# mkofinas/aether

Measured on AMD Instinct MI355X. Metric: edge-messages/sec (forward, electrostatic N=20 batch=128 per GPU), higher is better.
Workload: dtype f32; 1 GPU; electrostatic-2d-N20-B128; num_dims=2, nodes_per_graph=20, graphs_per_gpu=128, edges_per_gpu=48640, hidden=64, launch=hipgraph (10 steps per replay), parallelism=graphs sharded over 1 rank(s), no forward collective

## Files before the change

aether_amd/csrc/fused.h:

```cpp
#pragma once
#include "common.h"

#ifndef AETHER_SUMS_SELECT
#define AETHER_SUMS_SELECT 0
#endif
#ifndef AETHER_LATE_WAIT_FIRST
#define AETHER_LATE_WAIT_FIRST 0
#endif

namespace {

constexpr int FUSED_MAX_NODES = 32;
constexpr int FUSED_MAX_EDGES = 384;
constexpr int FUSED_MAX_TILES = FUSED_MAX_EDGES / 16;
constexpr int LDU = 2 * H + 8;

constexpr int FUSED_WIMG = SPLIT_WIMG;
constexpr int FUSED_CBLK = 768;
constexpr int CB_B1 = 0;
constexpr int CB_B2 = 64;
constexpr int CB_B3 = 128;
constexpr int CB_B4 = 256;
constexpr int CB_B1N = 320;
constexpr int CB_OB3 = 384;
constexpr int CB_OB6 = 448;
constexpr int CB_OW6 = 512;
template <int NW, int ROUNDS> struct FusedLds {
    static constexpr int WSZ = FUSED_WIMG;
    static constexpr int WA = 0;
    static constexpr int WB = WA + WSZ;
    static constexpr int CBLK = WB + WSZ;
    static constexpr int XBUF = CBLK + 2 * FUSED_CBLK;
    static constexpr int NBUF = XBUF + FUSED_MAX_NODES * LDW;
    static constexpr int PS = NBUF + FUSED_MAX_NODES * LDW;
    static constexpr int PR = PS + FUSED_MAX_NODES * LDW;
    static constexpr int NINFO = PR + FUSED_MAX_NODES * LDW;
    static constexpr int PART_ROWS = ROUNDS == 3 ? FUSED_MAX_NODES + FUSED_MAX_TILES : 2 * FUSED_MAX_NODES + 16;
    static constexpr int PART_SPARE = AETHER_SUMS_SELECT ? 1 : 0;
    static constexpr int PART = NINFO + FUSED_MAX_NODES * 24;
    static constexpr int ARRIVED = PART + (PART_ROWS + PART_SPARE) * LDW;
    static constexpr int SCRATCH = ARRIVED + 4;
    static constexpr int FEAT_ROWS = 16 * (ROUNDS < 2 ? ROUNDS : 2);
    static constexpr int SCRATCH_SIZE =
        NW * FEAT_ROWS * LDF > NW * 16 * LDST ? NW * FEAT_ROWS * LDF : NW * 16 * LDST;
    static constexpr int TOTAL = SCRATCH + SCRATCH_SIZE;
    static constexpr int FIELD_Z = SCRATCH;
    static constexpr int FIELD_H1 = FIELD_Z + FUSED_MAX_NODES * 24;
    static constexpr int FIELD_H2 = FIELD_H1 + FUSED_MAX_NODES * 32;
    static constexpr int FIELD_F = FIELD_H2 + FUSED_MAX_NODES * 32;
    static constexpr int FIELD_W = FIELD_F + FUSED_MAX_NODES * 4;
    static constexpr int FW0 = FIELD_W;
    static constexpr int FW2 = FW0 + 32 * 22;
    static constexpr int FW4 = FW2 + 32 * 32;
    static constexpr int FB = FW4 + 3 * 32;
    static constexpr int FEMB = FB + 68;
    static constexpr int FIELD_END = FEMB + 48;
    static constexpr int FEAT = SCRATCH;
    static constexpr int WSTAGE = SCRATCH;
    static constexpr int UBUF = SCRATCH;
    static constexpr int OBUF1 = SCRATCH;
    static constexpr int OBUF2 = SCRATCH + FUSED_MAX_NODES * LDW;
    static_assert(FIELD_END <= TOTAL, "field scratch");
    static_assert(UBUF + FUSED_MAX_NODES * LDU <= TOTAL, "ubuf");
    static_assert(OBUF2 + FUSED_MAX_NODES * LDW <= TOTAL, "obuf");
    static_assert(TOTAL * 4 <= 160 * 1024, "LDS budget");
};

constexpr int FUSED_NIMG_W3 = 2 * 8 * 2 * 64 * 4, FUSED_NIMG_W4 = 2 * 4 * 4 * 64 * 4, FUSED_NIMG_WS = 2 * 4 * 2 * 64 * 4;
constexpr int FUSED_NIMG_LAYER = FUSED_NIMG_W3 + FUSED_NIMG_W4 + 2 * FUSED_NIMG_WS;
constexpr int FUSED_WIMG_SET = 8 * FUSED_WIMG + 4 * FUSED_NIMG_LAYER + 4 * FUSED_CBLK;
constexpr int FUSED_SPLIT_BLOCKS = 8 + 4 * 6 + 1;
__device__ __host__ constexpr int fused_wimg_offset(int layer, int which) { return ((layer - 1) * 2 + which) * FUSED_WIMG; }
__device__ __host__ constexpr int fused_nimg_offset(int layer, int which) {
    return 8 * FUSED_WIMG + (layer - 1) * FUSED_NIMG_LAYER +
           (which == 0 ? 0 : which == 1 ? FUSED_NIMG_W3 : which == 2 ? FUSED_NIMG_W3 + FUSED_NIMG_W4 : FUSED_NIMG_W3 + FUSED_NIMG_W4 + FUSED_NIMG_WS);
}
__device__ __host__ constexpr int fused_cblk_offset(int layer) { return 8 * FUSED_WIMG + 4 * FUSED_NIMG_LAYER + (layer - 1) * FUSED_CBLK; }

__device__ __forceinline__ float fused_cblk_value(const AetherParams& P, int nd, int layer, int c) {
    if (c < CB_B2) return layer == 1 ? P.l1_msg_b0[c] : 0.0f;
    if (c < CB_B3) return (layer == 1 ? P.l1_msg_b2 : P.ln_msg_b2[layer - 2])[c - CB_B2];
    if (c < CB_B4) return (layer == 1 ? P.l1_upd_b0 : P.ln_upd_b0[layer - 2])[c - CB_B3];
    if (c < CB_B1N) return (layer == 1 ? P.l1_upd_b2 : P.ln_upd_b2[layer - 2])[c - CB_B4];
    if (c < CB_OB3) return (layer < 4 ? P.ln_msg_b0[layer - 1] : P.out_b0)[c - CB_B1N];
    if (layer < 4) return 0.0f;
    if (c < CB_OB6) return P.out_b3[c - CB_OB3];
    if (c < CB_OB6 + 4) return c - CB_OB6 < nd ? P.out_b6[c - CB_OB6] : 0.0f;
    if (c >= CB_OW6 && c < CB_OW6 + nd * H) return P.out_w6[c - CB_OW6];
    return 0.0f;
}

__device__ __forceinline__ void split_weights_block(const AetherParams& P, int f1, int nd, float* __restrict__ wimg, int block, int tid) {
    if (block == FUSED_SPLIT_BLOCKS - 1) {
        for (int idx = tid; idx < 4 * FUSED_CBLK; idx += 512)
            wimg[fused_cblk_offset(1) + idx] = fused_cblk_value(P, nd, idx / FUSED_CBLK + 1, idx % FUSED_CBLK);
        return;
    }
    if (block >= 8) {
        const int nbk = block - 8, layer = nbk / 6 + 1, part = nbk % 6;
        if (part < 2) {
            const float* w3 = layer == 1 ? P.l1_upd_w0 : P.ln_upd_w0[layer - 2];
            float* img = wimg + fused_nimg_offset(layer, 0);
#pragma unroll
            for (int j = 0; j < 2; ++j) {
                const int idx = tid + 512 * j, rr = 64 * part + (idx >> 4), cc = (idx & 15) * 4;
                stage_split4<8, 2>(img, rr, cc, ld4(w3 + (size_t)rr * H + cc));
            }
        } else if (part < 4) {
            const float* w4 = layer == 1 ? P.l1_upd_w2 : P.ln_upd_w2[layer - 2];
            float* img = wimg + fused_nimg_offset(layer, 1);
#pragma unroll
            for (int j = 0; j < 2; ++j) {
                const int idx = tid + 512 * j, rr = 32 * (part - 2) + (idx >> 5), cc = (idx & 31) * 4;
                stage_split4<4, 4>(img, rr, cc, ld4(w4 + (size_t)rr * (2 * H) + cc));
            }
        } else {
            const float* src = layer < 4 ? P.ln_msg_w0[layer - 1] + (part == 4 ? 0 : H) : (part == 4 ? P.out_w0 : P.out_w3);
            const int ld = layer < 4 ? 3 * H : H;
            float* img = wimg + fused_nimg_offset(layer, part - 2);
#pragma unroll
            for (int j = 0; j < 2; ++j) {
                const int idx = tid + 512 * j, rr = idx >> 4, cc = (idx & 15) * 4;
                stage_split4<4, 2>(img, rr, cc, ld4(src + (size_t)rr * ld + cc));
            }
        }
        return;
    }
    const int layer = block / 2 + 1, which = block & 1;
    float* img = wimg + fused_wimg_offset(layer, which);
    if (which == 0 && layer == 1) {
        const int r = tid >> 3, c0 = (tid & 7) * 4;
        f32x4 v;
#pragma unroll
        for (int b = 0; b < 4; ++b) v[b] = c0 + b < f1 ? P.l1_msg_w0[r * f1 + c0 + b] : 0.0f;
        stage_split4<4, 1>(img, r, c0, v);
        return;
    }
    const float* src;
    int ld;
    if (which == 0) { src = P.ln_msg_w0[layer - 2] + 2 * H; ld = 3 * H; }
    else { src = layer == 1 ? P.l1_msg_w2 : P.ln_msg_w2[layer - 2]; ld = H; }
#pragma unroll
    for (int j = 0; j < 2; ++j) {
        const int idx = tid + 512 * j, rr = idx >> 4, cc = (idx & 15) * 4;
        stage_split4<4, 2>(img, rr, cc, ld4(src + (size_t)rr * ld + cc));
    }
}

struct FusedDebug {
    float* nodeinfo; float* x[5]; float* e[4];
    float* n[4]; float* ps[3]; float* pr[3]; float* feat;
    int* flags;
    int* errword;
    const float* wimg;
    float* stamps;
    StepExtras step;
};
constexpr int FUSED_STAMPS = 512;

#ifdef AETHER_FUSED_STAMPS
// ... 84 lines not shown
    const int lane = threadIdx.x, i = lane & 15, q = lane >> 4;
    const int local = 16 * T.t + i;
    const bool valid = local < m;
    const int rcv = valid ? recv_s[eb + lorder[eb + local]] - wg.nb : -1;
    const int next = __shfl_down(rcv, 1, 16);
    const bool ends = valid && (i == 15 || next != rcv || local + 1 == na);
    const unsigned emask = (unsigned)__ballot(q == 0 && ends) & 0xFFFFu;
    const int second = (wg.partner >= 0 && local >= na) ? n : 0;
    const int myrow = rcv + T.t + second;
    const int j = lane & (FUSED_TREC - 1);
    unsigned w = 0;
#pragma unroll
    for (int b = 0; b < 4; ++b) {
        const int seg = 4 * (j - 2) + b;
        unsigned mm = emask;
        for (int t = 0; t < seg && mm != 0; ++t) mm &= mm - 1;
        const bool exists = seg >= 0 && seg < 16 && mm != 0;
        const int k = mm != 0 ? __ffs(mm) - 1 : 0;
        const int row = __shfl(myrow, k);
        w |= (exists ? (unsigned)row & 0xFFu : 0xFFu) << (8 * b);
    }
    if (j == 0) w = emask;
    if (j == 1) w = (unsigned)__popc(emask);
    if (j >= 6) w = 0;
    if (lane < FUSED_TREC) trec[(size_t)blockIdx.x * FUSED_TREC + lane] = w;
}

__device__ inline void graph_gtile(const int32_t* __restrict__ recv_s, int64_t n_edges, uint32_t* __restrict__ gsel,
                                   int64_t tile, int lane) {
    const int i = lane & 15, q = lane >> 4;
    const int64_t k = tile * 16 + i;
    const bool valid = k < n_edges;
    const int rcv = valid ? recv_s[k] : -1;
    const int prev = __shfl_up(rcv, 1, 16);
    const unsigned smask = (unsigned)__ballot(q == 0 && i > 0 && rcv != prev) & 0xFFFFu;
    const unsigned vmask = (unsigned)__ballot(q == 0 && valid) & 0xFFFFu;
    unsigned w = 0;
#pragma unroll
    for (int s4 = 0; s4 < 4; ++s4) {
        const int edge = 4 * s4 + q;
        const int seg_of_edge = __popc(smask & ((2u << edge) - 1u));
        if (((vmask >> edge) & 1u) && seg_of_edge == i) w |= 1u << s4;
    }
#pragma unroll
    for (int r4 = 0; r4 < 4; ++r4) {
        const int seg = 4 * q + r4;
        unsigned mm = smask;
        int s0 = 0;
        bool exists = true;
        for (int t = 0; t < seg; ++t) {
            if (mm == 0) { exists = false; break; }
            s0 = __ffs(mm) - 1;
            mm &= mm - 1;
        }
        const unsigned ok = (exists && ((vmask >> s0) & 1u)) ? 16u : 0u;
        w |= ((unsigned)s0 | ok) << (4 + 5 * r4);
    }
    gsel[(size_t)tile * 64 + lane] = w;
}

__global__ void __launch_bounds__(64)
k_graph_gtiles(const int32_t* __restrict__ recv_s, int64_t n_edges, uint32_t* __restrict__ gsel) {
    graph_gtile(recv_s, n_edges, gsel, (int64_t)blockIdx.x, threadIdx.x);
}

constexpr int GRAN_ROW = H * 8, GRAN_NODE = 3 * GRAN_ROW;
typedef unsigned int gran_u32x4 __attribute__((ext_vector_type(4)));

__device__ __forceinline__ auto gran_rsrc(int* flags, int goff, int vb, int nv) {
    return __builtin_amdgcn_make_buffer_rsrc(reinterpret_cast<char*>(flags) + goff + (int64_t)vb * GRAN_NODE, 0, nv * GRAN_NODE,
                                             0x00020000);
}

template <class Rsrc>
__device__ __forceinline__ void gran_publish(Rsrc rsrc, int row, int c0, int layer, f32x4 val) {
    const unsigned tag = (unsigned)layer;
    const gran_u32x4 g01 = {tag, __float_as_uint(val[0]), tag, __float_as_uint(val[1])};
    const gran_u32x4 g23 = {tag, __float_as_uint(val[2]), tag, __float_as_uint(val[3])};
    const int voff = row * GRAN_NODE + c0 * 8, soff = (layer - 1) * GRAN_ROW;
    __builtin_amdgcn_raw_buffer_store_b128(g01, rsrc, voff, soff, 16);
    __builtin_amdgcn_raw_buffer_store_b128(g23, rsrc, voff + 16, soff, 16);
}

template <class Rsrc, class LdsWord>
__device__ __forceinline__ void gran_receive(Rsrc rsrc, int layer, int nv, int n, int off, int lane, float* psb,
                                             LdsWord* arrived, int* errword) {
    constexpr int NL = 5;
    const int npieces = (nv - n) * (H / 2);
    const unsigned tag = (unsigned)(layer - 1);
    const int soff = (layer - 2) * GRAN_ROW;
    for (int base = 0; base < npieces; base += 64 * NL) {
        int src[NL];
#pragma unroll
        for (int j = 0; j < NL; ++j) {
            const int idx = base + 64 * j + lane, idc = idx < npieces ? idx : 0;
            int slot = idc >> 5;
            if (slot >= off) slot += n;
            src[j] = slot * GRAN_NODE + (idc & 31) * 16;
        }
        gran_u32x4 v[NL];
        unsigned spins = 0;
        unsigned long long t_first = 0;
        bool gave_up = false;
        for (;;) {
            asm volatile("" ::: "memory");
#pragma unroll
            for (int j = 0; j < NL; ++j) v[j] = __builtin_amdgcn_raw_buffer_load_b128(rsrc, src[j], soff, 16);
            __builtin_amdgcn_sched_barrier(0);
            __builtin_amdgcn_s_waitcnt(0x0F70);
            __builtin_amdgcn_sched_barrier(0);
            bool ok = true;
#pragma unroll
            for (int j = 0; j < NL; ++j) {
                asm volatile("" : "+v"(v[j]));
                ok = ok && v[j][0] == tag && v[j][2] == tag;
            }
            if (__all(ok)) break;
            __builtin_amdgcn_s_sleep(1);
            if ((++spins & 1023u) == 0) {
                const unsigned long long now = wall_clock64();
                if (t_first == 0) t_first = now;
                if (now - t_first <= 500000000ull) continue;
                if (lane == 0) {
                    if (errword) __hip_atomic_store(errword, 1, __ATOMIC_RELAXED, __HIP_MEMORY_SCOPE_SYSTEM);
                    arrived[1] = 1;
                }
                gave_up = true;
                break;
            }
        }
#pragma unroll
        for (int j = 0; j < NL; ++j) {
            if (base + 64 * j + lane < npieces) {
                const int row = src[j] / GRAN_NODE, c = ((src[j] % GRAN_NODE) >> 4) * 2;
                *reinterpret_cast<f32x2*>(psb + row * LDW + c) = f32x2{__uint_as_float(v[j][1]), __uint_as_float(v[j][3])};
            }
        }
        if (gave_up) break;
    }
}

template <class Rsrc>
__device__ __forceinline__ void gran_rearm(Rsrc rsrc, int nv, int n, int off, int t, int nthreads) {
    constexpr int PIECES = GRAN_NODE / 16;
    const gran_u32x4 zero = {0u, 0u, 0u, 0u};
    for (int idx = t; idx < (nv - n) * PIECES; idx += nthreads) {
        int slot = idx / PIECES;
        const int piece = idx - slot * PIECES;
        if (slot >= off) slot += n;
        __builtin_amdgcn_raw_buffer_store_b128(zero, rsrc, slot * GRAN_NODE + piece * 16, 0, 16);
    }
}

#ifndef AETHER_R3_DEFER
#define AETHER_R3_DEFER 0
#endif
template <int D, int NW, int ROUNDS, bool KEEP, bool GRAN = false>
__global__ void __launch_bounds__(NW * 64)
k_fused(AetherParams P, const float* __restrict__ x, const float* __restrict__ vel,
        const float* __restrict__ charges, const float* __restrict__ edge_attr_orig,
        const int32_t* __restrict__ perm, const int32_t* __restrict__ send_s,
        const int32_t* __restrict__ recv_s, const int32_t* __restrict__ rowptr,
        const FusedWG* __restrict__ wgdesc, const uint32_t* __restrict__ trec, const int4* __restrict__ ledge,
        const int32_t* __restrict__ nrange, FusedDebug dbg, float* __restrict__ out) {
    constexpr bool keep = KEEP;
    using NI = NodeInfo<D>;
    using L = FusedLds<NW, ROUNDS>;
    constexpr int THREADS = NW * 64;
    constexpr int FIN = 2 * D + 16;
    static_assert(NW == 8 || NW == 12, "waves 0-7 run the node phase; NW == 12 adds four waves that run step 3 (DESIGN.md 4.1)");
    static_assert(NW == 8 || (ROUNDS == 1 && !KEEP), "the 12-wave kernel owns one tile per wave and saves nothing for the backward");
    static_assert(!GRAN || NW == 12, "granules are the 12-wave kernel's hand-off");
    extern __shared__ __attribute__((aligned(16))) float smem[];
    float* wA = smem + L::WA;
    float* wB = smem + L::WB;
    const float* cblk = smem + L::CBLK;
    float* xbuf = smem + L::XBUF;
    float* nbuf = smem + L::NBUF;
    float* psb = smem + L::PS;
    float* prb = smem + L::PR;
    float* ninfo = smem + L::NINFO;
    float* part = smem + L::PART;

    const int tid = threadIdx.x, lane = tid & 63, wave = tid >> 6;
    const int i = lane & 15, q = lane >> 4;
    const FusedWG wg = wgdesc[blockIdx.x];
    const int vb = wg.vb, nv = wg.ve - wg.vb;
    const int nb = wg.nb, ne = wg.ne;
    const int n = ne - nb, off = nb - vb;
    const int eb = wg.eb, m = wg.m;
    const int n_tiles = (m + 15) >> 4;
    const int na = wg.na;
    typedef __attribute__((address_space(3))) volatile int lds_word;
    lds_word* arrived = (lds_word*)(smem + L::ARRIVED);
    if (tid == 0) { arrived[0] = 0; arrived[1] = 0; }
#ifdef AETHER_FUSED_STAMPS
    const unsigned long long t_entry = wall_clock64();
    const unsigned long long c_entry = __builtin_amdgcn_s_memtime();
#endif
    FUSED_STAMP(0);

    auto dma_images = [&](int layer_) {
        const int na_frag = layer_ == 1 ? 8 : 16, nw_frag = na_frag + 16;
        const int total = nw_frag + FUSED_CBLK / 256;
        const int wv = __builtin_amdgcn_readfirstlane(wave);
        __builtin_assume(wv >= 0 && wv < NW);
        const int g_img = fused_wimg_offset(layer_, 0), g_cb = fused_cblk_offset(layer_);
        const int l_cb = L::CBLK + (layer_ & 1) * FUSED_CBLK;
        constexpr int MAXF = (32 + FUSED_CBLK / 256 + NW - 1) / NW;
#pragma unroll
        for (int j = 0; j < MAXF; ++j) {
            const int f = wv + NW * j;
            if (f < total) {
                const int img = f < na_frag ? f * 256 : FUSED_WIMG + (f - na_frag) * 256;
                const int soff = f < nw_frag ? g_img + img : g_cb + (f - nw_frag) * 256;
                const int doff = f < nw_frag ? L::WA + img : l_cb + (f - nw_frag) * 256;
                __builtin_amdgcn_global_load_lds(dbg.wimg + soff + lane * 4, (__attribute__((address_space(3))) void*)(smem + doff), 16, 0, 0);
            }
        }
    };
    dma_images(1);
    FUSED_STAMP(1);

    constexpr int FR = ROUNDS < 2 ? ROUNDS : 2;
    const int f_local = 16 * (NW * (lane >> 4) + wave) + (lane & 15);
    const bool f_have = lane < 16 * FR && f_local < m;
    int4 f_e = make_int4(0, 0, 0, 0);
    f32x2 f_ea = {0.0f, 0.0f};
    int4 t_e[ROUNDS];
    unsigned seg_ends[ROUNDS];
    unsigned seg_rows[ROUNDS][4];
    {
        const int wv = __builtin_amdgcn_readfirstlane(wave);
#pragma unroll
        for (int r = 0; r < ROUNDS; ++r) {
            const int stile = NW * r + wv;
            const uint32_t* rec = trec + (size_t)(wg.tile0 + (stile < n_tiles ? stile : 0)) * FUSED_TREC;
            seg_ends[r] = stile < n_tiles ? __builtin_amdgcn_readfirstlane(rec[0]) : 0u;
#pragma unroll
            for (int w = 0; w < 4; ++w) seg_rows[r][w] = __builtin_amdgcn_readfirstlane(rec[2 + w]);
        }
    }
    const int aslot = (tid >> 4) & (FUSED_MAX_NODES - 1), ac4 = (tid & 15) * 4;
    int4 nr_rec;
    const int4* own_desc = reinterpret_cast<const int4*>(wgdesc + blockIdx.x);
    const int4* le_base = m > 0 ? ledge + eb : own_desc;
    const int4* nr_base = n > 0 ? reinterpret_cast<const int4*>(nrange) + nb : own_desc;
    const float* ea_base = m > 0 ? edge_attr_orig : reinterpret_cast<const float*>(own_desc);
    const float* qattr = dbg.step.qattr;
    auto index_stage_a = [&]() {
        f_e = le_base[f_have ? f_local : 0];
#pragma unroll
        for (int r = 0; r < ROUNDS; ++r) {
            const int tile = NW * r + wave, local = 16 * tile + i;
            t_e[r] = le_base[local < m ? local : 0];
        }
        nr_rec = nr_base[aslot < n ? aslot : 0];
    };
    auto index_select = [&]() {
        if (!f_have) f_e = make_int4(0, 0, 0, 0);
#pragma unroll
        for (int r = 0; r < ROUNDS; ++r) {
            t_e[r].x = m > 0 ? t_e[r].x : 0; t_e[r].y = m > 0 ? t_e[r].y : vb;
            t_e[r].z = m > 0 ? t_e[r].z : nb; t_e[r].w = m > 0 ? t_e[r].w : 0;
        }
    };
    auto index_stage_b = [&]() -> f32x2 {
        f32x2 v;
        if (qattr) {
            v[0] = qattr[f_e.y]; v[1] = qattr[f_e.z];
        } else {
            const float* ea = ea_base + 2 * (int64_t)f_e.w;
            v[0] = ea[0]; v[1] = ea[1];
        }
        return v;
    };

    {
        const int vtiles = (nv + 15) >> 4;
        if (wave < vtiles) {
            const float* p_emb = P.field_emb; const float* p_w0 = P.field_w0; const float* p_b0 = P.field_b0;
            const float* p_w2 = P.field_w2; const float* p_b2 = P.field_b2; const float* p_w4 = P.field_w4;
            const float* p_b4 = P.field_b4; const float* p_rb = P.l1_res_b; const float* p_rw = P.l1_res_w;
            const float* p_ext = dbg.step.ext_field ? dbg.step.ext_field : x;
            asm volatile("" :: "s"(p_emb), "s"(p_w0), "s"(p_b0), "s"(p_w2), "s"(p_b2), "s"(p_w4), "s"(p_b4), "s"(p_rb),
                         "s"(p_rw), "s"(p_ext), "s"(x), "s"(vel), "s"(charges), "s"(le_base), "s"(nr_base), "s"(ea_base),
                         "s"(qattr));
            const int node = 16 * wave + i;
            const bool live = node < nv;
            const int64_t g = vb + (live ? node : 0);
            float pz[D], vz[D], ef[D];
#pragma unroll
            for (int d = 0; d < D; ++d) { pz[d] = x[g * D + d]; vz[d] = vel[g * D + d]; ef[d] = p_ext[g * D + d]; }
            const float ch = charges[g];
            float zc[6][3], a1[2][6];
#pragma unroll
            for (int s4 = 0; s4 < 6; ++s4) {
                const int k = 4 * s4 + q;
                const int ke = (k >= 2 * D && k < FIN) ? k - 2 * D : 0, kw = k < FIN ? k : 0;
#pragma unroll
                for (int c = 0; c < 3; ++c)
                    zc[s4][c] = (4 * s4 + 3 >= 2 * D && 4 * s4 < FIN) ? p_emb[c * 16 + ke] : 0.0f;
#pragma unroll
                for (int mb = 0; mb < 2; ++mb) a1[mb][s4] = 4 * s4 < FIN ? p_w0[(16 * mb + i) * FIN + kw] : 0.0f;
            }
            f32x4 w2f[2][2], w4f[2], acc1[2], acc2[2];
#pragma unroll
            for (int mb = 0; mb < 2; ++mb) {
                acc1[mb] = ld4(p_b0 + 16 * mb + 4 * q);
                acc2[mb] = ld4(p_b2 + 16 * mb + 4 * q);
#pragma unroll
                for (int a = 0; a < 2; ++a) w2f[mb][a] = ld4(p_w2 + (16 * mb + i) * 32 + 16 * a + 4 * q);
            }
#pragma unroll
            for (int a = 0; a < 2; ++a) w4f[a] = ld4(p_w4 + (i < D ? i : 0) * 32 + 16 * a + 4 * q);
            f32x4 acc3 = f32x4{0.f, 0.f, 0.f, 0.f};
#pragma unroll
            for (int r = 0; r < 4; ++r) acc3[r] = r < D ? p_b4[4 * q + r < D ? 4 * q + r : 0] : 0.0f;
            float ar[4][2];
            f32x4 acc0[4];
#pragma unroll
            for (int mb = 0; mb < 4; ++mb) {
                acc0[mb] = ld4(p_rb + 16 * mb + 4 * q);
#pragma unroll
                for (int s4 = 0; s4 < 2; ++s4)
// ... 148 lines not shown
                    for (int t = 0; t < NI::STRIDE; ++t) { njl[t] = nj[t]; nrl[t] = nr[t]; }
                    float eal[2];
                    if (dbg.step.qattr) {
                        float d2 = 0.0f;
#pragma unroll
                        for (int d = 0; d < D; ++d) {
                            const float df = njl[NI::P + d] - nrl[NI::P + d];
                            d2 += df * df;
                        }
                        eal[0] = r0 == 0 ? f_ea[0] * f_ea[1] : dbg.step.qattr[ks] * dbg.step.qattr[kr];
                        eal[1] = sqrtf(d2);
                    } else if (r0 == 0) {
                        eal[0] = f_ea[0]; eal[1] = f_ea[1];
                    } else {
                        const float* ea = edge_attr_orig + 2 * (int64_t)le.w;
                        eal[0] = ea[0]; eal[1] = ea[1];
                    }
                    edge_features<D>(njl, nrl, eal, o);
                } else {
#pragma unroll
                    for (int t = 0; t < FPAD; ++t) o[t] = 0.0f;
                }
#pragma unroll
                for (int t = 0; t < FPAD; t += 4)
                    st4(scratch + lane * LDF + t, f32x4{o[t], o[t + 1], o[t + 2], o[t + 3]});
            }
            __builtin_amdgcn_wave_barrier();
#pragma unroll
            for (int rr = 0; rr < PASS; ++rr) {
                const int r = r0 + rr;
                if (r < ROUNDS) {
                    e[r][0] = ld4(scratch + (16 * rr + i) * LDF + 4 * q);
                    e[r][1] = ld4(scratch + (16 * rr + i) * LDF + 16 + 4 * q);
                }
            }
            asm volatile("s_waitcnt lgkmcnt(0)" ::: "memory");
            __builtin_amdgcn_wave_barrier();
        }
#pragma unroll
        for (int r = 0; r < ROUNDS; ++r) {
            e[r][2] = f32x4{0.f, 0.f, 0.f, 0.f};
            e[r][3] = f32x4{0.f, 0.f, 0.f, 0.f};
            const int local = 16 * (NW * r + wave) + i;
            sl[r] = t_e[r].y - vb;
            rl[r] = t_e[r].z - nb;
            if constexpr (KEEP) {
                ke[r] = local < m ? t_e[r].x : -1;
                if (ke[r] >= 0) {
                    st4(dbg.feat + (int64_t)ke[r] * FPAD + 4 * q, e[r][0]);
                    st4(dbg.feat + (int64_t)ke[r] * FPAD + 16 + 4 * q, e[r][1]);
                }
            }
        }
        lds_barrier();
    }
    FUSED_STAMP(3);

    unsigned arange = 0;
    float adeg = 1.0f;
    if constexpr (NW == 12) {
        asm volatile("" :: "v"(f_ea[0]), "v"(f_ea[1]), "v"(nr_rec.x), "v"(nr_rec.y), "v"(nr_rec.z), "v"(nr_rec.w));
    }
    if (aslot < n) {
        const int4 nr = nr_rec;
        const int at0 = nr.x >> 4;
        const int at1 = nr.y > nr.x ? ((nr.y - 1) >> 4) + 1 : at0;
        const int bt0 = (nr.z >> 4) + n;
        const int bt1 = nr.w > nr.z ? ((nr.w - 1) >> 4) + 1 + n : bt0;
        arange = (unsigned)at0 | (unsigned)at1 << 8 | (unsigned)bt0 << 16 | (unsigned)bt1 << 24;
        const int deg = (nr.y - nr.x) + (nr.w - nr.z);
        adeg = (float)(deg > 1 ? deg : 1);
    }

    f16x8 wsh[2], wsl[2], wrh[2], wrl[2];
    f16x8 wf_h[4], wf_l[4];
    const auto wimg_rsrc = __builtin_amdgcn_make_buffer_rsrc(const_cast<float*>(dbg.wimg), 0, FUSED_WIMG_SET * 4, 0x00020000);
    const int lane16 = lane * 16;
#pragma unroll 1
    for (int layer = 1; layer <= 4; ++layer) {
        const float* cb = cblk + (layer & 1) * FUSED_CBLK;
        const int mb2 = wave & 7;
        const int mb3 = wave & 3, tn3 = (wave >> 2) & 1;
        const bool act3 = wave < 8;
        const bool one_tile = NW == 12 ? true : n <= 16;
        const int tn4 = one_tile ? 0 : tn3;
        const int tn3s = tn4;
        const bool do3 = NW == 12 ? wave >= 8 : act3 && (one_tile ? wave >= 4 : 16 * tn3 < n);
        const bool do_s = act3 && (one_tile ? wave < 4 : true);
        const bool do_r = act3 && (one_tile ? wave >= 4 : true);
        f16x8 w3h[2], w3l[2], w4h[4], w4l[4];
        auto frag = [&](int block_bytes, int kb) -> f16x8 {
            return __builtin_bit_cast(f16x8, __builtin_amdgcn_raw_buffer_load_b128(wimg_rsrc, lane16, block_bytes + kb * 1024, 0));
        };
        auto load_frags = [&](int which, int mb, int MBN, int KBN, int kb0, int nkb, f16x8* wh, f16x8* wl) {
            if constexpr (ROUNDS == 3 && KEEP) {
                const f16x8* w = reinterpret_cast<const f16x8*>(dbg.wimg + fused_nimg_offset(layer, which)) +
                                 __builtin_amdgcn_readfirstlane(mb) * (KBN * 64);
#pragma unroll
                for (int kb = kb0; kb < kb0 + nkb; ++kb) {
                    wh[kb] = w[kb * 64 + lane];
                    wl[kb] = w[MBN * KBN * 64 + kb * 64 + lane];
                }
                return;
            }
            int lbytes = (layer - 1) * (FUSED_NIMG_LAYER * 4);
            asm volatile("" : "+s"(lbytes));
            const int blk = fused_nimg_offset(1, which) * 4 + lbytes + __builtin_amdgcn_readfirstlane(mb) * (KBN * 1024);
#pragma unroll
            for (int kb = kb0; kb < kb0 + nkb; ++kb) {
                wh[kb] = frag(blk, kb);
                wl[kb] = frag(blk + MBN * KBN * 1024, kb);
            }
        };
        auto issue_loads = [&](int part) {
            if constexpr (NW == 12) {
                const int wv = __builtin_amdgcn_readfirstlane(wave);
                int lbytes = (layer - 1) * (FUSED_NIMG_LAYER * 4);
                asm volatile("" : "+s"(lbytes));
                const bool w4 = wv >= 8;
                const int blk01 = lbytes + (w4 ? fused_nimg_offset(1, 1) * 4 + (wv & 3) * 4096 : fused_nimg_offset(1, 0) * 4 + wv * 2048);
                const int blk23 = w4 ? blk01 + 2048 : lbytes + (wv < 4 ? fused_nimg_offset(1, 2) : fused_nimg_offset(1, 3)) * 4 + (wv & 3) * 2048;
                const int lo23 = w4 ? 16 * 1024 : 8 * 1024;
                if (part == 1) {
#pragma unroll
                    for (int kb = 0; kb < 2; ++kb) {
                        wf_h[kb] = frag(blk01, kb);
                        wf_l[kb] = frag(blk01 + 16 * 1024, kb);
                    }
                }
                if (part == 3) {
#pragma unroll
                    for (int kb = 0; kb < 2; ++kb) {
                        wf_h[2 + kb] = frag(blk23, kb);
                        wf_l[2 + kb] = frag(blk23 + lo23, kb);
                    }
                }
            } else {
            if (part == 1 && act3) load_frags(0, mb2, 8, 2, 0, 2, w3h, w3l);
            if ((part == 2 || part == 3) && do3) load_frags(1, mb3, 4, 4, 2 * (part - 2), 2, w4h, w4l);
            if (part == 4 && (layer < 4 ? true : act3)) {
                if (layer == 4 || do_s) load_frags(2, mb3, 4, 2, 0, 2, wsh, wsl);
                if (layer == 4 || do_r) load_frags(3, mb3, 4, 2, 0, 2, wrh, wrl);
            }
            }
        };
        const bool xch = wg.partner >= 0 && layer > 1;
        auto front_gemm = [&](int r, f32x4 (&acc)[4], bool last, bool late_tile) {
            if (layer == 1) {
#pragma unroll
                for (int mb = 0; mb < 4; ++mb) acc[mb] = ld4(cb + CB_B1 + 16 * mb + 4 * q);
                f32x4 bop[2] = {e[r][0], e[r][1]};
                gemm_split<4, 1>(wA, bop, acc, lane);
            } else {
                f32x4 pr[4];
#pragma unroll
                for (int mb = 0; mb < 4; ++mb) {
                    pr[mb] = ld4(prb + rl[r] * LDW + 16 * mb + 4 * q);
                    acc[mb] = pr[mb] + ld4(psb + sl[r] * LDW + 16 * mb + 4 * q);
                }
                if (late_tile) {
                    const bool late = 16 * (NW * r + wave) + i >= na;
#pragma unroll
                    for (int mb = 0; mb < 4; ++mb)
#pragma unroll
                        for (int c = 0; c < 4; ++c) acc[mb][c] = late ? pr[mb][c] : acc[mb][c];
                }
                gemm_split<4, 2>(wA, e[r], acc, lane);
            }
        };
        auto late_add = [&](int r, f32x4 (&acc)[4]) {
            const bool late = 16 * (NW * r + wave) + i >= na;
            f32x4 ps[4];
#pragma unroll
            for (int mb = 0; mb < 4; ++mb) ps[mb] = ld4(psb + sl[r] * LDW + 16 * mb + 4 * q);
            asm volatile("s_waitcnt lgkmcnt(0)" : "+v"(ps[0]), "+v"(ps[1]), "+v"(ps[2]), "+v"(ps[3]));
#pragma unroll
            for (int mb = 0; mb < 4; ++mb)
#pragma unroll
                for (int c = 0; c < 4; ++c) acc[mb][c] = late ? acc[mb][c] + ps[mb][c] : acc[mb][c];
        };
        auto receive_partner_rows = [&]() {
            if constexpr (GRAN) {
                FUSED_WSTAMP(layer, 0, 6);
                gran_receive(gran_rsrc(dbg.flags, wg.goff, vb, nv), layer, nv, n, off, lane, psb, arrived, dbg.errword);
                asm volatile("s_waitcnt lgkmcnt(0)" ::: "memory");
                __builtin_amdgcn_wave_barrier();
                if (lane == 0) arrived[0] = layer;
                FUSED_WSTAMP(layer, 0, 7);
                return;
            }
            if (lane == 0) {
                unsigned spins = 0;
                unsigned long long t_first = 0;
                while (__hip_atomic_load(dbg.flags + wg.partner, __ATOMIC_RELAXED, __HIP_MEMORY_SCOPE_AGENT) < layer - 1) {
                    __builtin_amdgcn_s_sleep(2);
                    if ((++spins & 1023u) == 0) {
                        const unsigned long long now = wall_clock64();
                        if (t_first == 0) t_first = now;
                        if (now - t_first <= 500000000ull) continue;
                        if (dbg.errword) __hip_atomic_store(dbg.errword, 1, __ATOMIC_RELAXED, __HIP_MEMORY_SCOPE_SYSTEM);
                        arrived[1] = 1;
                        break;
                    }
                }
            }
            __builtin_amdgcn_fence(__ATOMIC_ACQUIRE, "wavefront");
            __builtin_amdgcn_wave_barrier();
            const int np = nv - n;
            typedef unsigned int u32x4 __attribute__((ext_vector_type(4)));
            const auto rsrc = __builtin_amdgcn_make_buffer_rsrc(dbg.ps[layer - 2] + (int64_t)vb * H, 0, nv * H * 4, 0x00020000);
            FUSED_WSTAMP(layer, 0, 6);
            if constexpr (NW == 12) {
                for (int base = 0; base < np * 16; base += 256) {
                    u32x4 v[4];
                    int dst[4];
#pragma unroll
                    for (int j = 0; j < 4; ++j) {
                        const int idx = base + 64 * j + lane, idc = idx < np * 16 ? idx : 0;
                        int slot = idc >> 4;
                        if (slot >= off) slot += n;
                        const int c = (idc & 15) * 4;
                        v[j] = __builtin_amdgcn_raw_buffer_load_b128(rsrc, (slot * H + c) * 4, 0, 16);
                        dst[j] = idx < np * 16 ? slot * LDW + c : -1;
                    }
                    __builtin_amdgcn_sched_barrier(0);
                    __builtin_amdgcn_s_waitcnt(0x0F70);
                    __builtin_amdgcn_sched_barrier(0);
#pragma unroll
                    for (int j = 0; j < 4; ++j) asm volatile("" :: "v"(v[j]));
#pragma unroll
                    for (int j = 0; j < 4; ++j) {
                        f32x4 f;
#pragma unroll
                        for (int r4 = 0; r4 < 4; ++r4) f[r4] = __uint_as_float(v[j][r4]);
                        if (dst[j] >= 0) st4(psb + dst[j], f);
                    }
                }
            } else
            for (int idx = lane; idx < np * 16; idx += 64) {
                int slot = idx >> 4;
                if (slot >= off) slot += n;
                const int c = (idx & 15) * 4;
                const u32x4 v = __builtin_amdgcn_raw_buffer_load_b128(rsrc, (slot * H + c) * 4, 0, 16);
                f32x4 f;
#pragma unroll
                for (int r4 = 0; r4 < 4; ++r4) f[r4] = __uint_as_float(v[r4]);
                st4(psb + slot * LDW + c, f);
            }
            asm volatile("s_waitcnt vmcnt(0) lgkmcnt(0)" ::: "memory");
            __builtin_amdgcn_wave_barrier();
            if (lane == 0) arrived[0] = layer;
            FUSED_WSTAMP(layer, 0, 7);
        };
        auto wait_partner_rows = [&]() {
            while (__builtin_amdgcn_readfirstlane(arrived[0]) < layer) __builtin_amdgcn_s_sleep(1);
            asm volatile("" ::: "memory");
        };
        auto front_act = [&](int r, f32x4 (&acc)[4], f32x4 (&h1)[4], bool last) {
            if (last && !(AETHER_R3_DEFER && ROUNDS >= 3)) issue_loads(1);
#pragma unroll
            for (int mb = 0; mb < 4; ++mb) h1[mb] = silu4(acc[mb]);
        };
        auto back = [&](int r, const f32x4 (&h1)[4], bool last) {
            const int tile = NW * r + wave;
            f32x4 acc2[4];
            if (last && !(AETHER_R3_DEFER && ROUNDS >= 3)) issue_loads(2);
#pragma unroll
            for (int mb = 0; mb < 4; ++mb) acc2[mb] = ld4(cb + CB_B2 + 16 * mb + 4 * q);
            gemm_split<4, 2>(wB, h1, acc2, lane);
            if (last && !(AETHER_R3_DEFER && ROUNDS >= 3)) issue_loads(3);
#pragma unroll
            for (int mb = 0; mb < 4; ++mb) e[r][mb] = silu4(acc2[mb]);
            if constexpr (KEEP) {
                if (ke[r] >= 0 && dbg.e[layer - 1] != nullptr) {
#pragma unroll
                    for (int mb = 0; mb < 4; ++mb)
                        st4(dbg.e[layer - 1] + (int64_t)ke[r] * H + 16 * mb + 4 * q, e[r][mb]);
                }
            }
            float* wst = smem + L::WSTAGE + wave * (16 * LDST);
#pragma unroll
            for (int mb = 0; mb < 4; ++mb) st4(wst + i * LDST + 16 * mb + 4 * q, e[r][mb]);
            FUSED_WSTAMP(layer, r, 4);
            __builtin_amdgcn_wave_barrier();
            {
                float cv[16];
#pragma unroll
                for (int k = 0; k < 16; ++k) cv[k] = wst[k * LDST + lane];
                float* pcol = part + lane;
                unsigned ends = seg_ends[r];
                asm volatile("" : "+s"(ends));
                unsigned long long lo = (unsigned long long)seg_rows[r][0] | ((unsigned long long)seg_rows[r][1] << 32);
                unsigned long long hi = (unsigned long long)seg_rows[r][2] | ((unsigned long long)seg_rows[r][3] << 32);
                float sum = 0.0f;
#pragma unroll
                for (int k = 0; k < 16; ++k) {
                    sum += cv[k];
#if AETHER_SUMS_SELECT
                    const bool end = (ends >> k) & 1u;
                    const unsigned row = end ? (unsigned)lo & 0xFFu : (unsigned)L::PART_ROWS;
                    pcol[row * LDW] = sum;
                    sum = end ? 0.0f : sum;
                    const unsigned long long nlo = (lo >> 8) | (hi << 56), nhi = hi >> 8;
                    lo = end ? nlo : lo;
                    hi = end ? nhi : hi;
#else
                    if ((ends >> k) & 1u) {
                        pcol[((unsigned)lo & 0xFFu) * LDW] = sum;
                        sum = 0.0f;
                        lo = (lo >> 8) | (hi << 56);
                        hi >>= 8;
                    }
#endif
                }
            }
            __builtin_amdgcn_wave_barrier();
            if (last && !(AETHER_R3_DEFER && ROUNDS >= 3)) issue_loads(4);
        };
        {
            const int nvalid = n_tiles > wave ? (n_tiles - wave + NW - 1) / NW : 0;
            if (nvalid == 0) {
#pragma unroll
                for (int part = 1; part < 5; ++part) issue_loads(part);
            }
            const int recv_wave = GRAN && na >= 16 ? 0 : NW - 1;
            if (xch && wave == recv_wave) receive_partner_rows();
            bool have_rows = !xch || wave == recv_wave;
#pragma unroll
            for (int r = 0; r < ROUNDS; ++r) {
                if (r < nvalid) {
                    const bool last = r == nvalid - 1;
                    const bool partner_tile = xch && 16 * (NW * r + wave + 1) > na;
                    constexpr bool LATE = NW == 12 || ROUNDS == 2;
                    const bool late_tile = LATE && partner_tile;
                    FUSED_WSTAMP(layer, r, 0);
                    if constexpr (!LATE || AETHER_LATE_WAIT_FIRST) {
                        if (partner_tile && !have_rows) {
                            wait_partner_rows();
                            have_rows = true;
                        }
                    }
                    FUSED_WSTAMP(layer, r, 1);
                    f32x4 acc[4], h1[4];
                    front_gemm(r, acc, last, late_tile);
                    FUSED_WSTAMP(layer, r, 3);
                    if (late_tile) {
                        if (!have_rows) {
                            wait_partner_rows();
                            have_rows = true;
                        }
                        FUSED_WSTAMP_ROWS(layer, r);
                        late_add(r, acc);
                    }
                    front_act(r, acc, h1, last);
                    FUSED_WSTAMP(layer, r, 2);
                    back(r, h1, last);
                    FUSED_WSTAMP(layer, r, 5);
                }
            }
            if constexpr (AETHER_R3_DEFER && ROUNDS >= 3) {
                if (nvalid > 0) { issue_loads(1); issue_loads(2); issue_loads(3); issue_loads(4); }
            }
        }
        FUSED_STAMP(4 + 8 * (layer - 1) + 2);
        lds_barrier();
        FUSED_STAMP(4 + 8 * (layer - 1) + 3);
        if (tid < FUSED_MAX_NODES * 16) {
            f32x4 sum = f32x4{0.f, 0.f, 0.f, 0.f};
            const int at0 = arange & 0xFF, at1 = (arange >> 8) & 0xFF, bt0 = (arange >> 16) & 0xFF, bt1 = arange >> 24;
            for (int t = at0; t < at1; ++t) sum += ld4(part + (aslot + t) * LDW + ac4);
            for (int t = bt0; t < bt1; ++t) sum += ld4(part + (aslot + t) * LDW + ac4);
            const f32x4 nv = ld4(xbuf + aslot * LDW + ac4) + sum / adeg;
            st4(nbuf + aslot * LDW + ac4, nv);
            if (keep && aslot < n) st4(dbg.n[layer - 1] + (int64_t)(nb + aslot) * H + ac4, nv);
        }
        __builtin_amdgcn_s_waitcnt(0x0F70);
        if (layer < 4) dma_images(layer + 1);
        lds_barrier();
        FUSED_STAMP(4 + 8 * (layer - 1) + 7);
        if (act3) {
            float* ubuf = smem + L::UBUF;
            const f32x4 bv = ld4(cb + CB_B3 + 16 * mb2 + 4 * q);
#pragma unroll
            for (int tn = 0; tn < 2; ++tn) {
                if (16 * tn < n) {
                    f32x4 nv[4];
#pragma unroll
                    for (int a = 0; a < 4; ++a) nv[a] = ld4(nbuf + (16 * tn + i) * LDW + 16 * a + 4 * q);
                    f32x4 acc;
                    if constexpr (NW == 12) {
                        const f16x8 wh2[2] = {wf_h[0], wf_h[1]}, wl2[2] = {wf_l[0], wf_l[1]};
                        acc = gemm_split_regs<2>(wh2, wl2, nv, bv);
                    } else {
                        acc = gemm_split_regs<2>(w3h, w3l, nv, bv);
                    }
                    st4(ubuf + (16 * tn + i) * LDU + 16 * mb2 + 4 * q, silu4(acc));
                }
            }
        }
        lds_barrier();
        FUSED_STAMP(4 + 8 * (layer - 1) + 4);

        if (do3) {
            const float* ubuf = smem + L::UBUF;
            f32x4 acc = ld4(cb + CB_B4 + 16 * mb3 + 4 * q);
#pragma unroll
            for (int hk = 0; hk < 2; ++hk) {
                f32x4 uv[4];
#pragma unroll
                for (int a = 0; a < 4; ++a) uv[a] = ld4(ubuf + (16 * tn3s + i) * LDU + 16 * (4 * hk + a) + 4 * q);
                if constexpr (NW == 12) {
                    const f16x8 wh2[2] = {wf_h[2 * hk], wf_h[2 * hk + 1]}, wl2[2] = {wf_l[2 * hk], wf_l[2 * hk + 1]};
                    acc = gemm_split_regs<2>(wh2, wl2, uv, acc);
                } else {
                    const f16x8 wh2[2] = {w4h[2 * hk], w4h[2 * hk + 1]}, wl2[2] = {w4l[2 * hk], w4l[2 * hk + 1]};
                    acc = gemm_split_regs<2>(wh2, wl2, uv, acc);
                }
            }
            acc += ld4(nbuf + (16 * tn3s + i) * LDW + 16 * mb3 + 4 * q);
            st4(xbuf + (16 * tn3s + i) * LDW + 16 * mb3 + 4 * q, acc);
            if (keep && 16 * tn3s + i < n)
                st4(dbg.x[layer] + (int64_t)(nb + 16 * tn3s + i) * H + 16 * mb3 + 4 * q, acc);
        }
        lds_barrier();
        FUSED_STAMP(4 + 8 * (layer - 1) + 5);
        if (layer < 4) {
            if constexpr (GRAN) __builtin_amdgcn_s_waitcnt(0x0F70);
            if (16 * tn4 < n) {
                f32x4 xv[4];
#pragma unroll
                for (int a = 0; a < 4; ++a) xv[a] = ld4(xbuf + (16 * tn4 + i) * LDW + 16 * a + 4 * q);
                if (do_s) {
                    f32x4 accs;
                    if constexpr (NW == 12) {
                        const f16x8 wh2[2] = {wf_h[2], wf_h[3]}, wl2[2] = {wf_l[2], wf_l[3]};
                        accs = gemm_split_regs<2>(wh2, wl2, xv, f32x4{0.f, 0.f, 0.f, 0.f});
                    } else {
                        accs = gemm_split_regs<2>(wsh, wsl, xv, f32x4{0.f, 0.f, 0.f, 0.f});
                    }
                    if (16 * tn4 + i < n) {
                        st4(psb + (off + 16 * tn4 + i) * LDW + 16 * mb3 + 4 * q, accs);
                        float* gps = dbg.ps[layer - 1] + (int64_t)(nb + 16 * tn4 + i) * H + 16 * mb3 + 4 * q;
                        if (GRAN && wg.partner >= 0) {
                            gran_publish(gran_rsrc(dbg.flags, wg.goff, vb, nv), off + 16 * tn4 + i, 16 * mb3 + 4 * q, layer, accs);
                        } else if (wg.partner >= 0) {
                            typedef unsigned int u32x4 __attribute__((ext_vector_type(4)));
                            const auto rsrc = __builtin_amdgcn_make_buffer_rsrc(
                                dbg.ps[layer - 1] + (int64_t)nb * H, 0, n * H * 4, 0x00020000);
                            u32x4 bits;
#pragma unroll
                            for (int r4 = 0; r4 < 4; ++r4) bits[r4] = __float_as_uint(accs[r4]);
                            __builtin_amdgcn_raw_buffer_store_b128(bits, rsrc, ((16 * tn4 + i) * H + 16 * mb3 + 4 * q) * 4, 0, 16);
                        } else if (keep) {
                            st4(gps, accs);
                        }
                    }
                }
                if (do_r) {
                    f32x4 accr;
                    if constexpr (NW == 12) {
                        const f16x8 wh2[2] = {wf_h[2], wf_h[3]}, wl2[2] = {wf_l[2], wf_l[3]};
                        accr = gemm_split_regs<2>(wh2, wl2, xv, ld4(cb + CB_B1N + 16 * mb3 + 4 * q));
                    } else {
                        accr = gemm_split_regs<2>(wrh, wrl, xv, ld4(cb + CB_B1N + 16 * mb3 + 4 * q));
                    }
                    st4(prb + (16 * tn4 + i) * LDW + 16 * mb3 + 4 * q, accr);
                    if (keep && 16 * tn4 + i < n)
                        st4(dbg.pr[layer - 1] + (int64_t)(nb + 16 * tn4 + i) * H + 16 * mb3 + 4 * q, accr);
                }
            }
            if (!GRAN)
                asm volatile("s_waitcnt vmcnt(0)" ::: "memory");
            lds_barrier();
            if (!GRAN && wg.partner >= 0 && tid == 0)
                __hip_atomic_store(dbg.flags + blockIdx.x, layer, __ATOMIC_RELAXED, __HIP_MEMORY_SCOPE_AGENT);
            FUSED_STAMP(4 + 8 * (layer - 1) + 6);
        }
    }
    if (wg.partner >= 0 && tid == 0)
        __hip_atomic_store(dbg.flags + wg.partner, 0, __ATOMIC_RELAXED, __HIP_MEMORY_SCOPE_AGENT);
    if constexpr (GRAN) {
        if (wg.partner >= 0 && wave >= 8) gran_rearm(gran_rsrc(dbg.flags, wg.goff, vb, nv), nv, n, off, tid - 512, 256);
    }

    {
        float* o1 = smem + L::OBUF1;
        float* o2 = smem + L::OBUF2;
        const int mb = wave & 3, tn = NW == 12 ? 0 : (wave >> 2) & 1;
        const bool act = wave < 8 && 16 * tn < n;
        const bool act1 = NW == 12 ? wave < 4 && n > 0 : act;
        const bool act2 = NW == 12 ? wave >= 4 && wave < 8 && n > 0 : act;
        const float* cb = cblk;
        if (act1) {
            f32x4 xv[4];
#pragma unroll
            for (int a = 0; a < 4; ++a) xv[a] = ld4(xbuf + (16 * tn + i) * LDW + 16 * a + 4 * q);
            f32x4 acc;
            if constexpr (NW == 12) {
                const f16x8 wh2[2] = {wf_h[2], wf_h[3]}, wl2[2] = {wf_l[2], wf_l[3]};
                acc = gemm_split_regs<2>(wh2, wl2, xv, ld4(cb + CB_B1N + 16 * mb + 4 * q));
            } else {
                acc = gemm_split_regs<2>(wsh, wsl, xv, ld4(cb + CB_B1N + 16 * mb + 4 * q));
            }
            f32x4 v = silu4(acc);
            if constexpr (KEEP) {
                if (dbg.step.drop1 != nullptr && 16 * tn + i < n)
                    v = v * ld4(dbg.step.drop1 + (int64_t)(nb + 16 * tn + i) * H + 16 * mb + 4 * q);
            }
            st4(o1 + (16 * tn + i) * LDW + 16 * mb + 4 * q, v);
        }
        if constexpr (KEEP) {
            if (blockIdx.x == 0 && tid == 0 && dbg.step.dropword != nullptr) *dbg.step.dropword = dbg.step.drop1 != nullptr ? 1 : 0;
        }
        lds_barrier();
        if (act2) {
            f32x4 xv[4];
#pragma unroll
            for (int a = 0; a < 4; ++a) xv[a] = ld4(o1 + (16 * tn + i) * LDW + 16 * a + 4 * q);
            f32x4 acc;
            if constexpr (NW == 12) {
                const f16x8 wh2[2] = {wf_h[2], wf_h[3]}, wl2[2] = {wf_l[2], wf_l[3]};
                acc = gemm_split_regs<2>(wh2, wl2, xv, ld4(cb + CB_OB3 + 16 * mb + 4 * q));
            } else {
                acc = gemm_split_regs<2>(wrh, wrl, xv, ld4(cb + CB_OB3 + 16 * mb + 4 * q));
            }
            f32x4 v = silu4(acc);
            if constexpr (KEEP) {
                if (dbg.step.drop2 != nullptr && 16 * tn + i < n)
                    v = v * ld4(dbg.step.drop2 + (int64_t)(nb + 16 * tn + i) * H + 16 * mb + 4 * q);
            }
            st4(o2 + (16 * tn + i) * LDW + 16 * mb + 4 * q, v);
        }
        lds_barrier();
        if (wave < 2 && 16 * wave < n) {
            const int tn2 = wave;
            f32x4 y = f32x4{0.f, 0.f, 0.f, 0.f};
#pragma unroll
            for (int a = 0; a < 4; ++a) {
                const f32x4 w6v = ld4(cb + CB_OW6 + (i < D ? i : D - 1) * H + 16 * a + 4 * q);
                const f32x4 xv = ld4(o2 + (16 * tn2 + i) * LDW + 16 * a + 4 * q);
#pragma unroll
                for (int b = 0; b < 4; ++b) y = mfma16(w6v[b], xv[b], y);
            }
            const int node = 16 * tn2 + i;
            if (q == 0 && node < n) {
                float yl[D];
#pragma unroll
                for (int d = 0; d < D; ++d) yl[d] = y[d] + cb[CB_OB6 + d];
                const float* ni = ninfo + (off + node) * 24;
#pragma unroll
                for (int a = 0; a < D; ++a) {
                    float s = 0.f;
#pragma unroll
                    for (int b = 0; b < D; ++b) s += ni[NI::R + a * D + b] * yl[b];
                    float xn = ni[NI::P + a] + s;
                    if (arrived[1]) xn = __builtin_nanf("");
                    out[(int64_t)(nb + node) * D + a] = xn;
                    if (dbg.step.vel_out)
                        dbg.step.vel_out[(int64_t)(nb + node) * D + a] = (xn - ni[NI::P + a]) / dbg.step.dt;
                }
            }
        }
    }
    FUSED_STAMP(40);
#ifdef AETHER_FUSED_STAMPS
    if (tid == 0 && blockIdx.x < 4096)
        dbg.stamps[blockIdx.x * FUSED_STAMPS + 41] = (float)(__builtin_amdgcn_s_memtime() - c_entry);
#endif
}

}
```

Measured before the change: 5.648 billion edge-messages/s.

## Precompute next layer's edge-weight product early to overlap node phase

In the 12-wave kernel, the next layer's W·e product for each wave's edge tile is computed ahead of time. Waves 0-7 do it after the node-phase barrier, and waves 8-11 do it during step 4. The front GEMM then only adds the sender and receiver sums. A new paired split-f16 MFMA routine interleaves weight-fragment loads with the MFMAs. The 8-wave LATE path now computes the product separately and adds the sums afterwards, which could change rounding slightly. It also moves where the waitcnt sits.

```diff
diff --git a/aether_amd/csrc/fused.h b/aether_amd/csrc/fused.h
--- a/aether_amd/csrc/fused.h
+++ b/aether_amd/csrc/fused.h
@@ -6,6 +6,9 @@
 #endif
 #ifndef AETHER_LATE_WAIT_FIRST
 #define AETHER_LATE_WAIT_FIRST 0
+#endif
+#ifndef AETHER_EARLY_PRODUCT
+#define AETHER_EARLY_PRODUCT 1
 #endif
 
 namespace {
@@ -396,6 +399,50 @@
     }
 }
 
+template <int MBN, int KBN>
+__device__ __forceinline__ void gemm_split_paired(const float* __restrict__ img, const f32x4 (&act)[2 * KBN], f32x4 (&acc)[MBN], int lane) {
+    static_assert(MBN % 2 == 0, "row blocks go in pairs");
+    constexpr int TERM = MBN * KBN * 64, NG = KBN * (MBN / 2);
+    const f16x8* w = reinterpret_cast<const f16x8*>(img);
+    const SplitScale sc = split_scale_of(act);
+    f32x4 x[2 * KBN];
+#pragma unroll
+    for (int b = 0; b < 2 * KBN; ++b) x[b] = act[b];
+    if (sc.on) {
+#pragma unroll
+        for (int b = 0; b < 2 * KBN; ++b) x[b] = x[b] * sc.s;
+#pragma unroll
+        for (int mb = 0; mb < MBN; ++mb) acc[mb] = acc[mb] * sc.s;
+    }
+    auto frag = [&](int g, int j, bool lo) -> f16x8 {
+        const int kb = g / (MBN / 2), mb = 2 * (g % (MBN / 2)) + j;
+        return w[(lo ? TERM : 0) + (mb * KBN + kb) * 64 + lane];
+    };
+    f16x8 xh[KBN], xl[KBN];
+    f16x8 wl0 = frag(0, 0, true), wl1 = frag(0, 1, true), wh0 = frag(0, 0, false), wh1 = frag(0, 1, false);
+    split8(x[0], x[1], xh[0], xl[0]);
+#pragma unroll
+    for (int g = 0; g < NG; ++g) {
+        const int kb = g / (MBN / 2), m0 = 2 * (g % (MBN / 2)), m1 = m0 + 1;
+        __builtin_amdgcn_sched_barrier(0);
+        acc[m0] = __builtin_amdgcn_mfma_f32_16x16x32_f16(wl0, xh[kb], acc[m0], 0, 0, 0);
+        acc[m1] = __builtin_amdgcn_mfma_f32_16x16x32_f16(wl1, xh[kb], acc[m1], 0, 0, 0);
+        __builtin_amdgcn_sched_barrier(0);
+        if (g + 1 < NG) { wl0 = frag(g + 1, 0, true); wl1 = frag(g + 1, 1, true); }
+        if (g + 1 < NG && (g + 1) % (MBN / 2) == 0) split8(x[2 * (kb + 1)], x[2 * (kb + 1) + 1], xh[kb + 1], xl[kb + 1]);
+        acc[m0] = __builtin_amdgcn_mfma_f32_16x16x32_f16(wh0, xl[kb], acc[m0], 0, 0, 0);
+        acc[m1] = __builtin_amdgcn_mfma_f32_16x16x32_f16(wh1, xl[kb], acc[m1], 0, 0, 0);
+        acc[m0] = __builtin_amdgcn_mfma_f32_16x16x32_f16(wh0, xh[kb], acc[m0], 0, 0, 0);
+        acc[m1] = __builtin_amdgcn_mfma_f32_16x16x32_f16(wh1, xh[kb], acc[m1], 0, 0, 0);
+        __builtin_amdgcn_sched_barrier(0);
+        if (g + 1 < NG) { wh0 = frag(g + 1, 0, false); wh1 = frag(g + 1, 1, false); }
+    }
+    if (sc.on) {
+#pragma unroll
+        for (int mb = 0; mb < MBN; ++mb) acc[mb] = acc[mb] * sc.inv_s;
+    }
+}
+
 #ifndef AETHER_R3_DEFER
 #define AETHER_R3_DEFER 0
 #endif
@@ -415,6 +462,8 @@
     static_assert(NW == 8 || NW == 12, "waves 0-7 run the node phase; NW == 12 adds four waves that run step 3 (DESIGN.md 4.1)");
     static_assert(NW == 8 || (ROUNDS == 1 && !KEEP), "the 12-wave kernel owns one tile per wave and saves nothing for the backward");
     static_assert(!GRAN || NW == 12, "granules are the 12-wave kernel's hand-off");
+    constexpr bool LATE = NW == 12 || ROUNDS == 2;
+    constexpr bool EARLY = NW == 12 && AETHER_EARLY_PRODUCT;
     extern __shared__ __attribute__((aligned(16))) float smem[];
     float* wA = smem + L::WA;
     float* wB = smem + L::WB;
@@ -869,20 +918,36 @@
                 f32x4 bop[2] = {e[r][0], e[r][1]};
                 gemm_split<4, 1>(wA, bop, acc, lane);
             } else {
-                f32x4 pr[4];
+                f32x4 pr[4], st[4];
 #pragma unroll
                 for (int mb = 0; mb < 4; ++mb) {
                     pr[mb] = ld4(prb + rl[r] * LDW + 16 * mb + 4 * q);
-                    acc[mb] = pr[mb] + ld4(psb + sl[r] * LDW + 16 * mb + 4 * q);
+                    st[mb] = pr[mb] + ld4(psb + sl[r] * LDW + 16 * mb + 4 * q);
                 }
                 if (late_tile) {
                     const bool late = 16 * (NW * r + wave) + i >= na;
 #pragma unroll
                     for (int mb = 0; mb < 4; ++mb)
 #pragma unroll
-                        for (int c = 0; c < 4; ++c) acc[mb][c] = late ? pr[mb][c] : acc[mb][c];
-                }
-                gemm_split<4, 2>(wA, e[r], acc, lane);
+                        for (int c = 0; c < 4; ++c) st[mb][c] = late ? pr[mb][c] : st[mb][c];
+                }
+                if constexpr (LATE) {
+                    if constexpr (EARLY) {
+#pragma unroll
+                        for (int mb = 0; mb < 4; ++mb) acc[mb] = e[r][mb] + st[mb];
+                    } else {
+                        f32x4 g[4];
+#pragma unroll
+                        for (int mb = 0; mb < 4; ++mb) g[mb] = f32x4{0.f, 0.f, 0.f, 0.f};
+                        gemm_split<4, 2>(wA, e[r], g, lane);
+#pragma unroll
+                        for (int mb = 0; mb < 4; ++mb) acc[mb] = g[mb] + st[mb];
+                    }
+                } else {
+#pragma unroll
+                    for (int mb = 0; mb < 4; ++mb) acc[mb] = st[mb];
+                    gemm_split<4, 2>(wA, e[r], acc, lane);
+                }
             }
         };
         auto late_add = [&](int r, f32x4 (&acc)[4]) {
@@ -972,6 +1037,16 @@
         auto wait_partner_rows = [&]() {
             while (__builtin_amdgcn_readfirstlane(arrived[0]) < layer) __builtin_amdgcn_s_sleep(1);
             asm volatile("" ::: "memory");
+        };
+        auto early_product = [&]() {
+            if (n_tiles > wave) {
+                f32x4 g[4];
+#pragma unroll
+                for (int mb = 0; mb < 4; ++mb) g[mb] = f32x4{0.f, 0.f, 0.f, 0.f};
+                gemm_split_paired<4, 2>(wA, e[0], g, lane);
+#pragma unroll
+                for (int mb = 0; mb < 4; ++mb) e[0][mb] = g[mb];
+            }
         };
         auto front_act = [&](int r, f32x4 (&acc)[4], f32x4 (&h1)[4], bool last) {
             if (last && !(AETHER_R3_DEFER && ROUNDS >= 3)) issue_loads(1);
@@ -1048,7 +1123,6 @@
                 if (r < nvalid) {
                     const bool last = r == nvalid - 1;
                     const bool partner_tile = xch && 16 * (NW * r + wave + 1) > na;
-                    constexpr bool LATE = NW == 12 || ROUNDS == 2;
                     const bool late_tile = LATE && partner_tile;
                     FUSED_WSTAMP(layer, r, 0);
                     if constexpr (!LATE || AETHER_LATE_WAIT_FIRST) {
@@ -1115,8 +1189,18 @@
                 }
             }
         }
+        if constexpr (EARLY) {
+            if (layer < 4) __builtin_amdgcn_s_waitcnt(0x0F70);
+        }
         lds_barrier();
         FUSED_STAMP(4 + 8 * (layer - 1) + 4);
+        if constexpr (EARLY) {
+            if (layer < 4 && wave < 8) {
+                FUSED_WSTAMP(layer + 1, 0, 8);
+                early_product();
+                FUSED_WSTAMP(layer + 1, 0, 9);
+            }
+        }
 
         if (do3) {
             const float* ubuf = smem + L::UBUF;
@@ -1142,7 +1226,14 @@
         lds_barrier();
         FUSED_STAMP(4 + 8 * (layer - 1) + 5);
         if (layer < 4) {
-            if constexpr (GRAN) __builtin_amdgcn_s_waitcnt(0x0F70);
+            if constexpr (GRAN && !EARLY) __builtin_amdgcn_s_waitcnt(0x0F70);
+            if constexpr (EARLY) {
+                if (wave >= 8) {
+                    FUSED_WSTAMP(layer + 1, 0, 8);
+                    early_product();
+                    FUSED_WSTAMP(layer + 1, 0, 9);
+                }
+            }
             if (16 * tn4 < n) {
                 f32x4 xv[4];
 #pragma unroll
```

Result: faster. 5.811 billion edge-messages/s (median of 6 runs) (+2.9%).
